# MiraPurkrabek/ProbPose_code

Measured on AMD Instinct MI355X. Metric: person-crops/sec @ 256x192 bs64, higher is better.
Workload: dtype f16x3

## Files before the change

include/probpose_mi355x.h:

```cpp
#ifndef PROBPOSE_MI355X_H_
#define PROBPOSE_MI355X_H_

#include <stddef.h>
#include <stdint.h>

#ifdef __cplusplus
extern "C" {
#endif

#define PP_ABI_VERSION 4


enum {
    PP_OK = 0,
    PP_ERR_INVALID_ARG = -1,
    PP_ERR_UNSUPPORTED = -2,
    PP_ERR_HIP = -3,
    PP_ERR_WORKSPACE = -4
};

#define PP_MAX_RADIUS 9
#define PP_MAX_TAPS (2 * PP_MAX_RADIUS + 1)

int pp_abi_version(void);
// ... 141 lines not shown

int pp_qkv_attention_split_folded(const void* x_centered, const void* wqkv_folded, const float* bqkv_folded, const float* ln_stats, void* out,
                                  int n_seq, int seq_len, int heads, int head_dim, float scale, float w_inv_scale, void* stream);

long long pp_proj_split_packed_bytes(int E);
int pp_proj_split_pack_weights(const void* wp_split, void* packed, int E, void* stream);
int pp_proj_ffn_split_residual_layernorm(const void* att, const void* wproj_packed, const float* bproj,
                                         const float* gamma2, const float* beta2, void* h_scratch, const void* w_packed,
                                         const float* b1, const float* b2, const float* residual, float* x_out,
                                         const float* gamma, const float* beta, float eps, void* h_out, int M, int E,
                                         int F, void* stream);
int pp_proj_ffn_split_residual_layernorm_ws(const void* att, const void* wproj_packed, const float* bproj,
                                            const float* gamma2, const float* beta2, void* h_scratch, const void* w_packed,
                                            const float* b1, const float* b2, const float* residual, float* x_out,
                                            const float* gamma, const float* beta, float eps, void* h_out, int M, int E,
                                            int F, float wp_inv_scale, float w1_inv_scale, float w2_inv_scale, void* stream);

int pp_proj_ffn_split_folded(const void* att, const void* wproj_packed, const float* bproj, const float* gamma2, const float* beta2,
                             void* h_scratch, const void* w_packed, const float* b1, const float* b2, const void* residual,
                             int residual_format, const float* residual_stats, int fold_out, float* x_out, const float* gamma,
                             const float* beta, float eps, void* h_out, float* stats_out, int M, int E, int F, float wp_inv_scale,
                             float w1_inv_scale, float w2_inv_scale, void* stream);

int pp_deconv_head(const void* act_nhwc, const void* weight, const float* bias, const void* head_w, const float* head_b,
                   float* logits_phased, int B, int H, int W, int Cin, int Cout, int K, void* stream);

int pp_deconv_head_split(const void* act_nhwc, const void* weight, const float* bias, const void* head_w_packed,
                         const float* head_b, float* logits_phased, int B, int H, int W, int Cin, int Cout, int K, void* stream);

int pp_probmap_head_decode_phased(const float* logits, const float* logits_flip, const int32_t* flip_indices,
                                  const double* taps, const int32_t* radius, int B, int K, int H, int W, double in_w,
                                  double in_h, float temperature, float normalize, float* avg_out, float* conv_out,
                                  float* locs, double* keypoints, float* scores, void* stream);

#define PP_DECODE_LOGITS 1
#define PP_DECODE_PHASED 2
#define PP_DECODE_SHIFT_HEATMAP 4
int pp_probmap_decode_flags(const float* maps, const float* maps_flip, const int32_t* flip_indices, const double* taps,
                            const int32_t* radius, int B, int K, int H, int W, double in_w, double in_h, float temperature,
                            float normalize, float* avg_out, float* conv_out, float* locs, double* keypoints, float* scores,
                            int flags, void* stream);

int pp_conv3x3_splitk(int prec, const void* act_nhwc, const void* weight, float* partials, int B, int H, int W, int Cin,
                      int Cout, int groups, long long stride_act_g, long long stride_w_g, int ksplit, void* stream);
int pp_sum_maxpool_relu_nhwc(const float* partials, int nsplit, long long split_stride, const float* bias,
                             int images_per_group, void* out, int out_bf16, int N, int H, int W, int C, int ph, int pw,
                             void* stream);

long long pp_winograd_scratch_bytes(int B, int H, int W, int Cin);
int pp_conv3x3_winograd_maxpool_relu(const void* act_nhwc, const void* u_packed, const float* bias, void* v_scratch,
                                     void* out_pooled, int B, int H, int W, int Cin, int Cout, int pool_h, int pool_w, int groups,
                                     void* stream);

int pp_tower_final(const void* feat, int feat_bf16, const float* w, const float* bias,
                   const int32_t* flip_indices, float* out, int B, int passes, int C, int K, float err_div,
                   void* stream);

int pp_extended_oks(const double* gt_kpts, const double* gt_bbox, const double* gt_area, const double* dt_kpts,
                    const double* sigmas, const int* gt_visibilities, int G, int D, int K, int n_vis,
                    double confidence_thr, double padding, int use_area, int original, double* out, void* stream);

int pp_pack_records(const double* keypoints, const float* scores, const float* scalars, double* records, int n, void* stream);

int pp_revert_heatmaps_max(const float* heatmaps, const double* inverse_maps, float* out, int n, int K, int hm_h, int hm_w,
                           int img_h, int img_w, void* stream);

int pp_heatmap_posterior(float* heatmaps, const float* presence, double* scratch, int K, int H, int W, void* stream);

int pp_exoks_cells(const double* gt_kpts, const double* gt_bbox, const double* gt_area, const double* dt_kpts,
                   const double* sigmas, const int* gt_visibilities, const int* cell_gt_off, const int* cell_dt_off,
                   const long long* cell_out_off, int n_cells, int K, int n_vis, double confidence_thr, double padding,
                   int use_area, int original, double* out, void* stream);

int pp_exoks_match(const double* ious, const int* cell_gt_off, const int* cell_dt_off, const long long* cell_iou_off,
                   const unsigned char* gt_ignore, const unsigned char* gt_iscrowd, const double* gt_area,
                   const double* gt_bbox, const double* dt_area, const double* dt_bbox, const double* area_rng,
                   const double* iou_thrs, int n_cells, int max_gt_per_cell, int N_gt, int N_dt, int L, int A, int T,
                   int match_by_bbox, int* dt_match, unsigned char* dt_ignore, int* gt_match,
                   unsigned char* gt_ignore_out, double* sim_sum, int* sim_cnt, void* stream);

int pp_exmap_accumulate(const int* dt_match, const unsigned char* dt_ignore, const unsigned char* gt_ignore,
                        const int* order, const double* dt_score, const double* rec_thrs, int n_cells, int N_gt, int N_dt,
                        int L, int A, int T, int R, int* chunk_scratch, double* precision, double* recall, double* scores,
                        void* stream);

int pp_warp_affine_u8(const void* img_hwc, int img_h, int img_w, int channels, const double* inverse_maps, void* crops_chw,
                      int n, int out_h, int out_w, void* stream);

long long pp_parea_scratch_bytes(int K, int H, int W);
int pp_parea_thresholds(const float* maps, int K, int H, int W, void* scratch, float* thr, int* draw, void* stream);
int pp_parea_compose(const void* image_rgb, int img_h, int img_w, int pad_left, int pad_top, const float* maps, int K,
                     const float* thr, const int* draw, const int* boxes, int n_boxes, void* canvas_rgb, int canvas_h,
                     int canvas_w, void* stream);
int pp_draw_poses(const void* image_rgb, int img_h, int img_w, const float* keypoints, const float* visible, const int* boxes,
                  int n, int K, const int* skeleton, const void* link_rgb, const void* kpt_rgb, int n_links, double kpt_thr,
                  float radius, float thickness, float alpha, void* out_rgb, void* stream);
int pp_resize_bilinear_u8(const void* src_rgb, int src_h, int src_w, void* dst_rgb, int dst_h, int dst_w, void* stream);

#ifdef __cplusplus
}
#endif
#endif
```

probpose_code_amd/_lib.py:

```python
import ctypes
import os
from ctypes import c_char_p, c_double, c_float, c_int, c_longlong, c_void_p

import torch

_HERE = os.path.dirname(os.path.abspath(__file__))
LIB_NAME = "libprobpose_mi355x.so"
LIB_PATH = os.path.join(_HERE, LIB_NAME)

PP_OK = 0
PP_ERR_INVALID_ARG = -1
PP_ERR_UNSUPPORTED = -2
PP_ERR_HIP = -3
PP_ERR_WORKSPACE = -4
PP_MAX_RADIUS = 9
PP_MAX_TAPS = 2 * PP_MAX_RADIUS + 1


class ProbPoseLibraryError(RuntimeError):

    def __init__(self, fn, status, message):
        super().__init__(f"{fn} failed with {status}: {message}")
        self.status = status

# ... 62 lines not shown
        [c_int, _P, _P, _P, _P, c_int, _P, _P, _P, c_float, _P, c_int, c_int, c_int, c_int, c_int, c_int, _P],
    ),
    "pp_gemm_residual_layernorm_ws": (
        c_int,
        [c_int, _P, _P, _P, _P, c_int, _P, _P, _P, c_float, _P, c_int, c_int, c_int, c_int, c_int, c_int, c_float, _P],
    ),
    "pp_mlp_residual_layernorm": (c_int, [_P, _P, _P, _P, _P, _P, _P, _P, _P, c_float, _P, c_int, c_int, c_int, _P]),
    "pp_proj_mlp_residual_layernorm": (
        c_int, [_P, _P, _P, _P, _P, _P, _P, _P, _P, _P, _P, _P, _P, c_float, _P, _P, _P, _P, c_int, c_int, c_int, _P]),
    "pp_vit_layer": (
        c_int, [_P, c_int, c_int, c_float, _P, _P, _P, _P, _P, _P, _P, _P, _P, _P, _P, _P, c_float, _P, _P, _P, _P, c_int, c_int,
                c_int, _P]),
    "pp_ffn_split_packed_bytes": (c_longlong, [c_int, c_int]),
    "pp_ffn_split_pack_weights": (c_int, [_P, _P, _P, c_int, c_int, _P]),
    "pp_ffn_split_residual_layernorm": (c_int, [_P, _P, _P, _P, _P, _P, _P, _P, c_float, _P, c_int, c_int, c_int, _P]),
    "pp_ffn_split_residual_layernorm_ws": (c_int, [_P, _P, _P, _P, _P, _P, _P, _P, c_float, _P, c_int, c_int, c_int, c_float, c_float, _P]),
    "pp_qkv_attention_split": (c_int, [_P, _P, _P, _P, c_int, c_int, c_int, c_int, c_float, _P]),
    "pp_qkv_attention_split_ws": (c_int, [_P, _P, _P, _P, c_int, c_int, c_int, c_int, c_float, c_float, _P]),
    "pp_qkv_attention_split_folded": (c_int, [_P] * 5 + [c_int] * 4 + [c_float, c_float, _P]),
    "pp_proj_split_packed_bytes": (c_longlong, [c_int]),
    "pp_proj_split_pack_weights": (c_int, [_P, _P, c_int, _P]),
    "pp_proj_ffn_split_residual_layernorm": (
        c_int, [_P, _P, _P, _P, _P, _P, _P, _P, _P, _P, _P, _P, _P, c_float, _P, c_int, c_int, c_int, _P]),
    "pp_proj_ffn_split_residual_layernorm_ws": (
        c_int, [_P, _P, _P, _P, _P, _P, _P, _P, _P, _P, _P, _P, _P, c_float, _P, c_int, c_int, c_int, c_float, c_float, c_float, _P]),
    "pp_proj_ffn_split_folded": (
        c_int, [_P] * 10 + [c_int, _P, c_int, _P, _P, _P, c_float, _P, _P, c_int, c_int, c_int, c_float, c_float, c_float, _P]),
    "pp_conv3x3_splitk": (c_int, [c_int, _P, _P, _P, c_int, c_int, c_int, c_int, c_int, c_int, c_longlong, c_longlong, c_int, _P]),
    "pp_sum_maxpool_relu_nhwc": (c_int, [_P, c_int, c_longlong, _P, c_int, _P, c_int, c_int, c_int, c_int, c_int, c_int, c_int, _P]),
    "pp_warp_affine_u8": (c_int, [_P, c_int, c_int, c_int, _P, _P, c_int, c_int, c_int, _P]),
    "pp_extended_oks": (
        c_int, [_P, _P, _P, _P, _P, _P, c_int, c_int, c_int, c_int, c_double, c_double, c_int, c_int, _P, _P]),
    "pp_pack_records": (c_int, [_P, _P, _P, _P, c_int, _P]),
    "pp_revert_heatmaps_max": (c_int, [_P, _P, _P] + [c_int] * 6 + [_P]),
    "pp_heatmap_posterior": (c_int, [_P, _P, _P, c_int, c_int, c_int, _P]),
    "pp_exoks_cells": (
        c_int, [_P] * 9 + [c_int, c_int, c_int, c_double, c_double, c_int, c_int, _P, _P]),
    "pp_exoks_match": (
        c_int, [_P] * 12 + [c_int] * 8 + [_P] * 7),
    "pp_exmap_accumulate": (
        c_int, [_P] * 6 + [c_int] * 7 + [_P] * 5),
    "pp_conv_gemm": (
        c_int,
        [c_int, c_int, _P, _P, _P, _P, c_int, c_int, c_int, c_int, c_int, c_int, c_int, c_int,
         c_longlong, c_longlong, c_longlong, c_longlong, c_int, c_int, c_int, _P],
    ),
    "pp_attention": (c_int, [c_int, _P, _P, c_int, c_int, c_int, c_int, c_float, _P]),
    "pp_preproc_im2col": (c_int, [c_int, _P, c_int, _P, c_int, c_int, c_int, c_int, c_int, c_int, _P, _P, c_int, _P]),
    "pp_layernorm": (c_int, [_P, _P, _P, _P, c_int, c_int, c_float, c_int, _P]),
    "pp_maxpool_relu_nhwc": (c_int, [_P, c_int, _P, c_int, c_int, c_int, c_int, c_int, c_int, c_int, _P]),
    "pp_conv3x3_maxpool_relu": (c_int, [c_int, _P, _P, _P, _P, _P] + [c_int] * 8 + [c_longlong] * 3 + [c_int, _P]),
    "pp_winograd_scratch_bytes": (c_longlong, [c_int] * 4),
    "pp_conv3x3_winograd_maxpool_relu": (c_int, [_P] * 5 + [c_int] * 8 + [_P]),
    "pp_tower_final": (c_int, [_P, c_int, _P, _P, _P, _P, c_int, c_int, c_int, c_int, c_float, _P]),
    "pp_parea_scratch_bytes": (c_longlong, [c_int, c_int, c_int]),
    "pp_parea_thresholds": (c_int, [_P, c_int, c_int, c_int, _P, _P, _P, _P]),
    "pp_parea_compose": (c_int, [_P, c_int, c_int, c_int, c_int, _P, c_int, _P, _P, _P, c_int, _P, c_int, c_int, _P]),
    "pp_draw_poses": (
        c_int, [_P, c_int, c_int, _P, _P, _P, c_int, c_int, _P, _P, _P, c_int, c_double, c_float, c_float, c_float, _P, _P]),
    "pp_resize_bilinear_u8": (c_int, [_P, c_int, c_int, _P, c_int, c_int, _P]),
}

for _name, (_res, _args) in SIGNATURES.items():
    _fn = getattr(lib, _name)
    _fn.restype = _res
    _fn.argtypes = _args


class PlanShape(ctypes.Structure):
    _fields_ = [(n, c_int) for n in ("prec", "n_img", "n_tokens", "embed", "ffn", "patch_k", "n_keypoints", "feat_h", "feat_w",
                                     "heat_h", "heat_w", "deconv_channels")]


WS = dict(patches=0, x=1, h=2, qkv=3, att=4, ln2=5, ffn=6, feat=7, logits=8, deconv=9, tower=10, tower_partial=11, tower_pooled=12, winograd=13, ln_stats=14)


def workspace_bytes(buffer: str, shape: "PlanShape", index: int = 0) -> int:
    n = lib.pp_workspace_bytes(WS[buffer], index, ctypes.byref(shape))
    if n < 0:
        raise ProbPoseLibraryError("pp_workspace_bytes", lib.pp_status_string(int(n)).decode(), last_error())
    return int(n)


_option_epoch = 0


_option_first_values = {}


def set_option(name: str, value: int) -> None:
    global _option_epoch
    if name not in _option_first_values:
        v = ctypes.c_int(0)
        if lib.pp_get_option(name.encode(), ctypes.byref(v)) == PP_OK:
            _option_first_values[name] = int(v.value)
    check("pp_set_option", lib.pp_set_option(name.encode(), int(value)))
    _option_epoch += 1


def restore_options() -> None:
    for name, v in list(_option_first_values.items()):
        if get_option(name) != v:
            set_option(name, v)


def option_epoch() -> int:
# ... 58 lines not shown
```

probpose_code_amd/engine.py:

```python
import math
import os
import warnings
from typing import Dict, Optional, Sequence

import numpy as np
import ctypes

import torch

from . import _lib
from .codecs import oks_kernel_taps
from .weights import PackedWeights, from_split, pack, to_split

PREC = {"bf16": 0, "f32": 1, "f16x3": 2}
_DTYPE = {"bf16": torch.bfloat16, "f32": torch.float32, "f16x3": torch.float32}
_FMT = {"bf16": 1, "f32": 0, "f16x3": 2}
ACT_NONE, ACT_GELU, ACT_RELU = 0, 1, 2
CONV3X3, DECONV = 1, 2


PLAN_DEFAULTS = dict(fuse_mlp=True, fuse_proj=True, fuse_qkv=True, split_k=True, fuse_attn=True, fuse_head=True, fuse_resln=None,
                     fuse_pool=True, fuse_qkv_attn=True, winograd=True, ln_fold=True, small_plan=True, head_two_streams=True)
SMALL_PLAN_ROWS_BELOW = 6912

# ... 99 lines not shown
            bp = torch.zeros(rows, dtype=torch.float32, device=fb.device)
            bp[: fb.shape[0]] = fb
            self._final_padded = (wp, bp)
        self.small_rows_below = SMALL_PLAN_ROWS_BELOW
        self.fuse_attn, self.fuse_head, self.fuse_pool = pl["fuse_attn"], pl["fuse_head"], pl["fuse_pool"]
        self.fuse_resln = pl["fuse_resln"] is not False
        self._resln_768 = pl["fuse_resln"] is True
        self._ffn_packed: Dict[int, torch.Tensor] = {}
        self._proj_packed: Dict[int, torch.Tensor] = {}
        if precision == "f16x3" and self.fuse_mlp and _lib.lib.pp_ffn_split_packed_bytes(self.E, self.w.ffn_dims) > 0:
            nbytes = _lib.lib.pp_ffn_split_packed_bytes(self.E, self.w.ffn_dims)
            pbytes = _lib.lib.pp_proj_split_packed_bytes(self.E) if self.fuse_proj else -1
            with torch.cuda.device(self.device):
                for i in range(self.w.num_layers):
                    buf = torch.empty(nbytes // 4, dtype=torch.float32, device=self.device)
                    _lib.call("pp_ffn_split_pack_weights", self.w[f"l{i}.fc1.w"].data_ptr(), self.w[f"l{i}.fc2.w"].data_ptr(),
                              buf.data_ptr(), self.E, self.w.ffn_dims, _lib.stream_ptr(self.device))
                    self._ffn_packed[i] = buf
                    if pbytes > 0:
                        pbuf = torch.empty(pbytes // 4, dtype=torch.float32, device=self.device)
                        _lib.call("pp_proj_split_pack_weights", self.w[f"l{i}.proj.w"].data_ptr(), pbuf.data_ptr(), self.E,
                                  _lib.stream_ptr(self.device))
                        self._proj_packed[i] = pbuf
                torch.cuda.synchronize(self.device)
            if not (pl["small_plan"]):
                for i in range(self.w.num_layers):
                    for name in (f"l{i}.fc1.w", f"l{i}.fc2.w") + ((f"l{i}.proj.w",) if i in self._proj_packed else ()):
                        self.w.t.pop(name, None)
        self.fuse_qkv_attn = precision == "f16x3" and pl["fuse_qkv_attn"] and self.Np == 192 and self.hd == 32 and self.E == 384
        self.ln_fold = bool(precision == "f16x3" and pl["ln_fold"] and not self._proj_packed and not self._ffn_packed
                            and self.w.has("l0.fc1.wf") and self.E % 192 == 0 and self.w.ffn_dims % 192 == 0)
        self.ln_fold_fused = bool(precision == "f16x3" and pl["ln_fold"] and self.fuse_qkv_attn and self._proj_packed and self.w.has("l1.qkv.wf")
                                  and (self.w.ffn_dims // 128) % 2 == 0 and self.w.num_layers >= 2)
        if precision == "f16x3":
            if self.fuse_qkv_attn and self._proj_packed:
                self.layer_plan = "two launches per layer (pp_qkv_attention_split + pp_proj_ffn_split_residual_layernorm)"
                if self.ln_fold_fused:
                    self.layer_plan += "; ln1 of layers 1 .. L - 1 folded into the qkv projection (pp_proj_ffn_split_folded -> pp_qkv_attention_split_folded)"
            elif self._proj_packed:
                self.layer_plan = "three launches per layer (pp_gemm qkv + pp_attention + pp_proj_ffn_split_residual_layernorm)"
            else:
                self.layer_plan = "generic (pp_gemm / pp_attention / pp_layernorm per layer)"
                if self.ln_fold:
                    self.layer_plan += ("; from the row count at which the twelve-wave Linear kernel engages: LayerNorm folded into the Linear "
                                        "layers (pp_linear_ln_folded x4 + pp_attention per layer, residual stream in the operand format)")
            if pl["fuse_qkv_attn"] and not self.fuse_qkv_attn and self.E == 384 and self.hd == 32:
                warnings.warn(
                    f"ProbPoseEngine: {self.Np}-token sequences ({img_size[0]}x{img_size[1]} input) miss the fused qkv + attention kernel, "
                    f"which is built for 192 tokens (256x192); this model runs {self.layer_plan}", RuntimeWarning, stacklevel=2)
        else:
            self.layer_plan = "bf16 / f32 plan"
        self.winograd = (precision == "f16x3" and pl["winograd"] and self.w.has("tower0.wino")
                         and _lib.lib.pp_winograd_scratch_bytes(1, self.Hp, self.Wp, self.E) > 0)
        if self.w.has("tower0.wino") and not self.winograd:
            self.w.t.pop("tower0.wino")
        self._logits_phased = False
        self._head_stream: Optional[torch.cuda.Stream] = None
        self._capture_events: list = []
        self._eager_events: dict = {}
        self.profile: Optional[Dict[str, list]] = None
        self.stage_hook = None
        self.pools = ((4, 3), (2, 2), (2, 2))
        hs, ws_ = self.Hp, self.Wp
        self.tower_hw = []
        for ph, pw_ in self.pools:
            self.tower_hw.append((hs, ws_))
            hs, ws_ = hs // ph, ws_ // pw_
        if (hs, ws_) != (1, 1):
            raise ValueError(
                f"scalar towers reduce the {self.Hp}x{self.Wp} feature map to {hs}x{ws_}; the reference "
                "reshapes them to (B, 1, K) (probmap_head.py:780-783), which needs 1x1"
            )

    def ksplit(self, nb: int, th: int, tw: int) -> int:
        return int(_lib.lib.pp_conv3x3_splitk_slices(self.prec, int(nb), int(th), int(tw), self.E, self.E, 4))

    def _workspace(self, B: int, passes: int, slot: int = 0) -> Dict[str, torch.Tensor]:
        self._check_options()
        key = (B, passes, slot)
        if key in self._ws:
            return self._ws[key]
        dev, T, f32 = self.device, self.dtype, torch.float32
        nb = B * passes
        M = nb * self.Np
        E, Fd = self.E, self.w.ffn_dims
        dc = self.w.deconv_channels
        shape = _lib.PlanShape(prec=self.prec, n_img=nb, n_tokens=self.Np, embed=E, ffn=Fd, patch_k=3 * self.P * self.P, n_keypoints=self.K,
                               feat_h=self.Hp, feat_w=self.Wp, heat_h=self.Hh, heat_w=self.Wh, deconv_channels=dc[0] if dc else 0)

        def buf(which, dims, dt=T, index=0):
            nbytes = _lib.workspace_bytes(which, shape, index)
            t = torch.empty(nbytes, dtype=torch.uint8, device=dev).view(dt)
            assert t.numel() == math.prod(dims), (which, index, nbytes, dims)
            return t.view(*dims)

        e = lambda *s, dt=T: torch.empty(s, dtype=dt, device=dev)
        small = self._small_at(M)
        fused_layer = self.precision == "f16x3" and self.fuse_qkv_attn and bool(self._proj_packed) and not small
        ws = dict(
            patches=buf("patches", (M, 3 * self.P * self.P)), x=buf("x", (M, E), f32), h=buf("h", (M, E)),
            feat=buf("feat", (M, E)), logits=buf("logits", (nb, self.K, self.Hh * self.Wh), f32),
            qkv=None if (fused_layer or (small and self.fuse_qkv_attn)) else buf("qkv", (M, 3 * E)),
            qkv2=None if (fused_layer or small) else buf("qkv", (M, 3 * E)),
            f=None if ((fused_layer or self._ffn_packed) and not small) else buf("ffn", (M, Fd)),
            att=buf("att", (M, E)) if (self.fuse_qkv_attn or small) else None,
            hs=buf("ln2", (M, E)) if (self._proj_packed or small) else None,
            ln_count=torch.zeros((M + 31) // 32, dtype=torch.int32, device=dev) if small else None,
            xs=buf("h", (M, E)) if self._ln_fold_at(M) else None,
# ... 243 lines not shown
            wj = w[f"deconv{j}.w"]
            if (j == nd - 1 and self.fuse_head and ob == 1 and cout == 256 and w.has("final.w_pad") and cin % 32 == 0
                    and ww % 4 == 0 and self.K <= 28):
                self._call("deconv_head", "pp_deconv_head", src.data_ptr(), wj.data_ptr(), w[f"deconv{j}.b"].data_ptr(),
                           w["final.w_pad"].data_ptr(), w["final.b"].data_ptr(), ws["logits"].data_ptr(), nb, hh, ww, cin, cout,
                           self.K, st)
                self._logits_phased = True
                return ws["logits"]
            if (j == nd - 1 and self.fuse_head and ob == 2 and cout == 256 and w.has("final.w_head") and cin % 32 == 0
                    and ww % 4 == 0 and self.K <= 28 and nb * hh * ww * 4 >= 192 * 192):
                self._call("deconv_head", "pp_deconv_head_split", src.data_ptr(), wj.data_ptr(), w[f"deconv{j}.b"].data_ptr(),
                           w["final.w_head"].data_ptr(), w["final.b"].data_ptr(), ws["logits"].data_ptr(), nb, hh, ww, cin, cout,
                           self.K, st)
                self._logits_phased = True
                return ws["logits"]
            if ob == 2 and self._small_at(nb * self.Np) and nb * hh * ww <= 1536 and cin % 32 == 0 and cout % 32 == 0:
                self._call("deconv", "pp_skinny_deconv", src.data_ptr(), wj.data_ptr(), w[f"deconv{j}.b"].data_ptr(), dst.data_ptr(), nb, hh, ww, cin,
                           cout, st)
                src, cin, hh, ww = dst, cout, hh * 2, ww * 2
                continue
            self._call("deconv", "pp_conv_gemm", self.prec, DECONV, src.data_ptr(), wj.data_ptr(),
                       w[f"deconv{j}.b"].data_ptr(), dst.data_ptr(), nb, hh, ww, cin, cout, -1, -1, 1, 0, 0, 0, 0, cout,
                       ACT_RELU, ob, st)
            src, cin, hh, ww = dst, cout, hh * 2, ww * 2
        P = hh * ww
        if ob == 2 and self._small_at(nb * self.Np) and cin % 64 == 0 and self._final_padded is not None:
            wp, bp = self._final_padded
            self._call("final_conv", "pp_skinny_conv1x1_planar", src.data_ptr(), wp.data_ptr(), bp.data_ptr(), ws["logits"].data_ptr(), nb, P, cin, self.K,
                       w.inv("final.w"), st)
            return ws["logits"]
        self._gemm(st, src, w["final.w"], w["final.b"], ws["logits"], nb * P, self.K, cin, planar=P, out_bf16=0)
        return ws["logits"]

    def towers(self, feat: torch.Tensor, B: int, passes: int, flip_indices, ws, st) -> torch.Tensor:
        w, E = self.w, self.E
        nb = B * passes
        ob = self.fmt
        src, stride_src = feat, 0
        for j, (th, tw) in enumerate(self.tower_hw):
            ph, pw_ = self.pools[j]
            out = ws[f"t{j}"]
            rows = nb * th * tw
            if self.split_k and f"tp{j}" in ws:
                part = ws[f"tp{j}"]
                ks = part.shape[0]
                self._call("conv3x3_splitk", "pp_conv3x3_splitk", self.prec, src.data_ptr(), w[f"tower{j}.w"].data_ptr(),
                           part.data_ptr(), nb, th, tw, E, E, 4, stride_src, E * 9 * E, ks, st)
                self._call("maxpool", "pp_sum_maxpool_relu_nhwc", part.data_ptr(), ks, 4 * rows * E, w[f"tower{j}.b"].data_ptr(),
                           nb, ws[f"p{j}"].data_ptr(), ob, 4 * nb, th, tw, E, ph, pw_, st)
                src = ws[f"p{j}"]
                stride_src = nb * (th // ph) * (tw // pw_) * E
                continue
            if j == 0 and self.winograd and ws.get("wino") is not None and stride_src == 0 and (ph, pw_) == (4, 3):
                self._call("conv3x3", "pp_conv3x3_winograd_maxpool_relu", src.data_ptr(), w["tower0.wino"].data_ptr(), w["tower0.b"].data_ptr(),
                           ws["wino"].data_ptr(), ws["p0"].data_ptr(), nb, th, tw, E, E, ph, pw_, 4, st)
            elif self.fuse_pool:
                self._call("conv3x3", "pp_conv3x3_maxpool_relu", self.prec, src.data_ptr(), w[f"tower{j}.w"].data_ptr(),
                           w[f"tower{j}.b"].data_ptr(), ws[f"p{j}"].data_ptr(), out.data_ptr(), nb, th, tw, E, E, ph, pw_, 4,
                           stride_src, E * 9 * E, E, ob, st)
            else:
                self._call("conv3x3", "pp_conv_gemm", self.prec, CONV3X3, src.data_ptr(), w[f"tower{j}.w"].data_ptr(),
                           w[f"tower{j}.b"].data_ptr(), out.data_ptr(), nb, th, tw, E, E, 0, 0, 4, stride_src,
                           E * 9 * E, nb * th * tw * E, E, E, ACT_NONE, ob, st)
                self._call("maxpool", "pp_maxpool_relu_nhwc", out.data_ptr(), ob, ws[f"p{j}"].data_ptr(), ob, 4 * nb, th, tw, E, ph,
                           pw_, st)
            src = ws[f"p{j}"]
            stride_src = nb * (th // ph) * (tw // pw_) * E
        fi = self._flip_indices(flip_indices) if passes == 2 else None
        self._call("tower_final", "pp_tower_final", src.data_ptr(), ob, w["tower_out.w"].data_ptr(), w["tower_out.b"].data_ptr(),
                  _lib.ptr(fi), ws["scalars"].data_ptr(), B, passes, E, self.K, 1.0, st)
        return ws["scalars"]

    def _check_imgs(self, imgs: torch.Tensor):
        assert imgs.dim() == 4 and imgs.is_cuda, "expects a (B,3,H,W) tensor on the GPU"
        assert imgs.dtype in (torch.uint8, torch.float32), "crops are uint8 (raw) or float32 (already preprocessed)"
        assert tuple(imgs.shape[1:]) == (3, self.H, self.W), f"crop shape {tuple(imgs.shape)} != (B,3,{self.H},{self.W})"

    @torch.no_grad()
    def run_backbone(self, imgs: torch.Tensor, flip_test: bool, slot: int = 0) -> torch.Tensor:
        self._check_imgs(imgs)
        imgs = imgs.contiguous()
        B, passes = imgs.shape[0], 2 if flip_test else 1
        ws = self._workspace(B, passes, slot)
        with torch.cuda.device(self.device):
            feat = self.backbone(imgs, passes, ws, _lib.stream_ptr(self.device))
        return feat.view(B * passes, self.Hp, self.Wp, self.E)

    def export_features(self, feat: torch.Tensor) -> torch.Tensor:
        return from_split(feat) if self.precision == "f16x3" else feat.clone()

    def import_features(self, x_nhwc: torch.Tensor) -> torch.Tensor:
        if self.precision == "f16x3":
            return to_split(x_nhwc.float().contiguous())
        if x_nhwc.dtype != self.dtype or not x_nhwc.is_contiguous():
            x_nhwc = x_nhwc.to(self.dtype).contiguous()
        return x_nhwc

    @torch.no_grad()
    def run_head(self, feat_nhwc: torch.Tensor, flip_test: bool, flip_indices=None,
                 return_heatmaps: bool = False, slot: int = 0, shift_heatmap: bool = False) -> Dict[str, torch.Tensor]:
        passes = 2 if flip_test else 1
        nb = feat_nhwc.shape[0]
        assert nb % passes == 0 and tuple(feat_nhwc.shape[1:]) == (self.Hp, self.Wp, self.E)
        assert feat_nhwc.dtype == self.dtype and feat_nhwc.is_contiguous() and feat_nhwc.is_cuda
        if flip_test and flip_indices is None:
            raise ValueError("flip_test needs flip_indices (dataset meta)")
        B = nb // passes
        ws = self._workspace(B, passes, slot)
# ... 171 lines not shown
```

probpose_code_amd/weights.py:

```python
import math
from dataclasses import dataclass, field
from typing import Dict, List

import torch

TOWERS = ("probability", "visibility", "oks", "error")
BN_EPS = 1e-5


def to_split(x: torch.Tensor) -> torch.Tensor:
    K = x.shape[-1]
    assert K % 32 == 0, f"split-fp16 tensors need a last dimension that is a multiple of 32, got {K}"
    x = x.float()
    hi = x.half()
    lo = (x - hi.float()).half()
    lead = x.shape[:-1]
    blocks = torch.stack([hi.reshape(*lead, K // 32, 32), lo.reshape(*lead, K // 32, 32)], dim=-2)
    return blocks.reshape(*lead, 2 * K).contiguous().view(torch.float32)


def from_split(c: torch.Tensor) -> torch.Tensor:
    K = c.shape[-1]
    v = c.contiguous().view(torch.float16).reshape(*c.shape[:-1], K // 32, 2, 32).float()
    return (v[..., 0, :] + v[..., 1, :]).reshape(c.shape)
# ... 72 lines not shown


@dataclass
class PackedWeights:
    dtype: torch.dtype
    embed_dims: int
    num_layers: int
    ffn_dims: int
    num_keypoints: int
    deconv_channels: List[int]
    t: Dict[str, torch.Tensor] = field(default_factory=dict)
    inv_scale: Dict[str, float] = field(default_factory=dict)

    def __getitem__(self, k):
        return self.t[k]

    def inv(self, k) -> float:
        return float(self.inv_scale.get(k, 1.0))

    def has(self, k) -> bool:
        return k in self.t


def _bn_fold(sd, name):
    scale = sd[name + ".weight"].float() / torch.sqrt(sd[name + ".running_var"].float() + BN_EPS)
    shift = sd[name + ".bias"].float() - sd[name + ".running_mean"].float() * scale
    return scale, shift


def pack_head_split(w32: torch.Tensor) -> torch.Tensor:
    assert tuple(w32.shape) == (32, 256)
    w32 = w32.float()
    hi = w32.half()
    lo = (w32 - hi.float()).half()
    lane = torch.arange(64)
    fr, fg = lane % 16, lane // 16
    j = torch.arange(8)
    ch_in_blk = torch.where(j < 4, 4 * fg[:, None] + j[None, :], 16 + 4 * fg[:, None] + (j[None, :] - 4))
    out = torch.empty((4, 2, 2, 2, 64, 8), dtype=torch.float16)
    for cg in range(4):
        for kb in range(2):
            ch = 64 * cg + 32 * kb + ch_in_blk
            for nf in range(2):
                rows = (16 * nf + fr)[:, None].expand(64, 8)
                out[cg, kb, nf, 0] = hi[rows, ch]
                out[cg, kb, nf, 1] = lo[rows, ch]
    return out.reshape(-1).view(torch.float32).contiguous()


def winograd_weights(w: torch.Tensor) -> torch.Tensor:
    G = torch.tensor([[1.0, 0.0, 0.0], [0.5, 0.5, 0.5], [0.5, -0.5, 0.5], [0.0, 0.0, 1.0]], dtype=torch.float64)
    u = torch.einsum("ai,ocij,bj->aboc", G, w.double(), G)
    return u.reshape(16, w.shape[0], w.shape[1]).float()


def pack(sd: Dict[str, torch.Tensor], dtype: torch.dtype, device, split: bool = False, scale_linear: bool = True,
         num_heads: int = 0, fold_ln: bool = True) -> PackedWeights:
    sd = {k: v.detach().cpu() for k, v in normalize_state_dict(sd).items()}
    if split and scale_linear and num_heads > 0:
        n_layers = 1 + max(int(k.split(".")[2]) for k in sd if k.startswith("backbone.layers."))
        for i in range(n_layers):
            if sd[f"backbone.layers.{i}.attn.qkv.weight"].shape[1] % num_heads == 0:
                balance_attention_dims(sd, f"backbone.layers.{i}.", num_heads)
    f32 = lambda x: x.float().contiguous().to(device)
    inv_scale: Dict[str, float] = {}
    if split:
        def op(x, name="weights", scaled=False):
            check_split_range(name, x)
            x = x.float()
            if scaled and scale_linear:
                e = weight_scale_exponent(x)
                x = x * 2.0 ** e
                inv_scale[name] = 2.0 ** -e
            return to_split(x.contiguous()).to(device)
    else:
        op = lambda x, name=None, scaled=False: x.float().contiguous().to(dtype).to(device)
    pw = sd["backbone.patch_embed.projection.weight"]
    E = pw.shape[0]
    L = 1 + max(int(k.split(".")[2]) for k in sd if k.startswith("backbone.layers."))
    Fd = sd["backbone.layers.0.ffn.layers.0.0.weight"].shape[0]
    K = sd["head.final_layer.weight"].shape[0]
    t: Dict[str, torch.Tensor] = {}
    t["patch_w"] = op(pw.reshape(E, -1), "patch_w")
    t["patch_b"] = f32(sd["backbone.patch_embed.projection.bias"])
    t["pos_embed"] = f32(sd["backbone.pos_embed"].reshape(-1, E))
    for i in range(L):
        p = f"backbone.layers.{i}."
        for ln in ("ln1", "ln2"):
            t[f"l{i}.{ln}.w"] = f32(sd[p + ln + ".weight"])
            t[f"l{i}.{ln}.b"] = f32(sd[p + ln + ".bias"])
        t[f"l{i}.qkv.w"] = op(sd[p + "attn.qkv.weight"], f"l{i}.qkv.w", scaled=True)
        qb = sd.get(p + "attn.qkv.bias")
        t[f"l{i}.qkv.b"] = f32(qb if qb is not None else torch.zeros(3 * E))
        t[f"l{i}.proj.w"] = op(sd[p + "attn.proj.weight"], f"l{i}.proj.w", scaled=True)
        t[f"l{i}.proj.b"] = f32(sd[p + "attn.proj.bias"])
        t[f"l{i}.fc1.w"] = op(sd[p + "ffn.layers.0.0.weight"], f"l{i}.fc1.w", scaled=True)
        t[f"l{i}.fc1.b"] = f32(sd[p + "ffn.layers.0.0.bias"])
        t[f"l{i}.fc2.w"] = op(sd[p + "ffn.layers.1.weight"], f"l{i}.fc2.w", scaled=True)
        t[f"l{i}.fc2.b"] = f32(sd[p + "ffn.layers.1.bias"])
        if split and fold_ln and E == 384 and i >= 1:
            bb = sd.get(p + "attn.qkv.bias")
            e = weight_scale_exponent(sd[p + "attn.qkv.weight"].double() * sd[p + "ln1.weight"].double()[None, :]) if scale_linear else 0
            wf, _, bf = fold_layernorm(sd[p + "attn.qkv.weight"].float(), bb.float() if bb is not None else torch.zeros(3 * E),
                                       sd[p + "ln1.weight"].float(), sd[p + "ln1.bias"].float(), name=f"l{i}.qkv.wf", scale_exp=e)
            t[f"l{i}.qkv.wf"], t[f"l{i}.qkv.bf"] = wf.to(device), bf.to(device)
            inv_scale[f"l{i}.qkv.wf"] = 2.0 ** -e
        if split and fold_ln and E % 192 == 0 and E != 384:
            for name, wk, bk, ln in (("qkv", "attn.qkv.weight", "attn.qkv.bias", "ln1"), ("fc1", "ffn.layers.0.0.weight", "ffn.layers.0.0.bias", "ln2")):
                bb = sd.get(p + bk)
                e = weight_scale_exponent(sd[p + wk].double() * sd[p + ln + ".weight"].double()[None, :]) if scale_linear else 0
                wf, cs, bf = fold_layernorm(sd[p + wk].float(), bb.float() if bb is not None else torch.zeros(sd[p + wk].shape[0]),
                                            sd[p + ln + ".weight"].float(), sd[p + ln + ".bias"].float(), name=f"l{i}.{name}.wf", scale_exp=e)
                t[f"l{i}.{name}.wf"], t[f"l{i}.{name}.cf"], t[f"l{i}.{name}.bf"] = wf.to(device), cs.to(device), bf.to(device)
                inv_scale[f"l{i}.{name}.wf"] = 2.0 ** -e
    t["ln_f.w"] = f32(sd["backbone.ln1.weight"])
    t["ln_f.b"] = f32(sd["backbone.ln1.bias"])

    deconv_channels = []
    j = 0
    while f"head.deconv_layers.{3 * j}.weight" in sd:
        w = sd[f"head.deconv_layers.{3 * j}.weight"].float()
        assert w.shape[2:] == (4, 4), "only deconv kernel 4 / stride 2 / pad 1 (the ProbPose config) is packed"
        scale, shift = _bn_fold(sd, f"head.deconv_layers.{3 * j + 1}")
        w = w * scale.view(1, -1, 1, 1)
        cin, cout = w.shape[:2]
        ph = torch.empty((2, 2, cout, 4 * cin))
        for py in range(2):
            for px in range(2):
                for ty in range(2):
                    for tx in range(2):
                        tap = ty * 2 + tx
                        ph[py, px, :, tap * cin : (tap + 1) * cin] = w[:, :, 3 - 2 * ty - py, 3 - 2 * tx - px].t()
        t[f"deconv{j}.w"] = op(ph, f"deconv{j}.w")
        t[f"deconv{j}.b"] = f32(shift)
        deconv_channels.append(cout)
        j += 1
    t["final.w"] = op(sd["head.final_layer.weight"].reshape(K, -1), "final.w")
    t["final.b"] = f32(sd["head.final_layer.bias"])
    if K <= 32:
        wpad = torch.zeros((32, t["final.w"].shape[1]), dtype=torch.float32)
        wpad[:K] = sd["head.final_layer.weight"].reshape(K, -1).float()
        t["final.w_pad"] = op(wpad, "final.w_pad")
        if split and wpad.shape[1] == 256:
            t["final.w_head"] = pack_head_split(wpad).to(device)

    for c in range(3):
        ws, bs, wino = [], [], []
        for tw in TOWERS:
            base = f"head.{tw}_layers."
            w = sd[base + f"{4 * c}.weight"].float()
            b = sd[base + f"{4 * c}.bias"].float()
            scale, shift = _bn_fold(sd, base + f"{4 * c + 1}")
            w = w * scale.view(-1, 1, 1, 1)
            ws.append(w.permute(0, 2, 3, 1).reshape(w.shape[0], -1))
            bs.append(b * scale + shift)
            if c == 0 and split:
                wino.append(winograd_weights(w))
        if c == 0 and split and w.shape[1] % 128 == 0 and w.shape[0] % 96 == 0:
            t["tower0.wino"] = op(torch.stack(wino), "tower0.wino")
        t[f"tower{c}.w"] = op(torch.stack(ws), f"tower{c}.w")
        t[f"tower{c}.b"] = f32(torch.stack(bs))
    t["tower_out.w"] = f32(torch.stack([sd[f"head.{tw}_layers.12.weight"].float().reshape(K, -1) for tw in TOWERS]))
    t["tower_out.b"] = f32(torch.stack([sd[f"head.{tw}_layers.12.bias"].float() for tw in TOWERS]))
    return PackedWeights(dtype=dtype, embed_dims=E, num_layers=L, ffn_dims=Fd, num_keypoints=K,
                         deconv_channels=deconv_channels, t=t, inv_scale=inv_scale)
```

Before: 14700.

## Add Winograd F(4x3,3x3) conv with fused maxpool for first tower layer

Adds a new Winograd variant whose output tile matches the (4,3) maxpool window, using 30 transform points instead of 16 per 2x2 tile. The output transform is folded into the GEMM epilogue so each pooled output is produced directly. The intent is fewer multiplies per output pixel and less scratch traffic for the first tower conv than the existing F(2x2) path. The trade-offs are larger transform coefficients with a numerical accuracy risk in split-f16 precision, and more accumulator registers.

```diff
diff --git a/include/probpose_mi355x.h b/include/probpose_mi355x.h
--- a/include/probpose_mi355x.h
+++ b/include/probpose_mi355x.h
@@ -217,6 +217,11 @@
                                      void* out_pooled, int B, int H, int W, int Cin, int Cout, int pool_h, int pool_w, int groups,
                                      void* stream);
 
+long long pp_winograd43_scratch_bytes(int B, int H, int W, int Cin);
+int pp_conv3x3_winograd43_maxpool_relu(const void* act_nhwc, const void* u_packed, const float* bias, void* v_scratch,
+                                       void* out_pooled, int B, int H, int W, int Cin, int Cout, int pool_h, int pool_w, int groups,
+                                       void* stream);
+
 int pp_tower_final(const void* feat, int feat_bf16, const float* w, const float* bias,
                    const int32_t* flip_indices, float* out, int B, int passes, int C, int K, float err_div,
                    void* stream);
diff --git a/probpose_code_amd/_lib.py b/probpose_code_amd/_lib.py
--- a/probpose_code_amd/_lib.py
+++ b/probpose_code_amd/_lib.py
@@ -138,6 +138,8 @@
     "pp_conv3x3_maxpool_relu": (c_int, [c_int, _P, _P, _P, _P, _P] + [c_int] * 8 + [c_longlong] * 3 + [c_int, _P]),
     "pp_winograd_scratch_bytes": (c_longlong, [c_int] * 4),
     "pp_conv3x3_winograd_maxpool_relu": (c_int, [_P] * 5 + [c_int] * 8 + [_P]),
+    "pp_winograd43_scratch_bytes": (c_longlong, [c_int] * 4),
+    "pp_conv3x3_winograd43_maxpool_relu": (c_int, [_P] * 5 + [c_int] * 8 + [_P]),
     "pp_tower_final": (c_int, [_P, c_int, _P, _P, _P, _P, c_int, c_int, c_int, c_int, c_float, _P]),
     "pp_parea_scratch_bytes": (c_longlong, [c_int, c_int, c_int]),
     "pp_parea_thresholds": (c_int, [_P, c_int, c_int, c_int, _P, _P, _P, _P]),
diff --git a/probpose_code_amd/csrc/pp_winograd43.hip b/probpose_code_amd/csrc/pp_winograd43.hip
--- /dev/null
+++ b/probpose_code_amd/csrc/pp_winograd43.hip
@@ -0,0 +1,341 @@
+#include "pp_common.h"
+#include "pp_split.h"
+
+namespace pp {
+namespace wino43 {
+
+typedef float f32x4 __attribute__((ext_vector_type(4)));
+typedef unsigned int u32x4 __attribute__((ext_vector_type(4)));
+typedef __attribute__((address_space(3))) void* lds_ptr_t;
+
+constexpr int PH = 4, PW = 3;
+constexpr int NP = 30;
+constexpr int RF = 2, CF = 3;
+constexpr int BT = 32 * RF, BN = 32 * CF, THREADS = 256;
+constexpr int NST = 4;
+constexpr unsigned OOB = 0x7ffffff0u;
+
+struct Params {
+    const void* V;
+    const void* U;
+    const float* bias;
+    void* out;
+    int T, Cin, Cout, groups;
+    int order;
+    unsigned v_bytes, u_bytes;
+};
+
+__device__ __forceinline__ f32x4 mma(const u32x4& a, const u32x4& b, f32x4 c) {
+    return __builtin_amdgcn_mfma_f32_16x16x32_f16(__builtin_bit_cast(f16x8, a), __builtin_bit_cast(f16x8, b), c, 0, 0, 0);
+}
+
+template <int N>
+__device__ __forceinline__ void wait_vm_lgkm() {
+    __builtin_amdgcn_s_waitcnt((N & 15) | (7 << 4) | (0 << 8) | ((N >> 4) << 14));
+}
+
+__device__ __forceinline__ float atr(int i, int a) {
+    if (a == 0) return i == 0 ? 1.f : 0.f;
+    if (a == 5) return i == 3 ? 1.f : 0.f;
+    const float x = a == 1 ? 1.f : (a == 2 ? -1.f : (a == 3 ? 0.5f : -0.5f));
+    return i == 0 ? 1.f : (i == 1 ? x : (i == 2 ? x * x : x * x * x));
+}
+__device__ __forceinline__ float atc(int j, int b) {
+    if (b == 0) return j == 0 ? 1.f : 0.f;
+    if (b == 4) return j == 2 ? 1.f : 0.f;
+    const float x = b == 1 ? 1.f : (b == 2 ? -1.f : 0.5f);
+    return j == 0 ? 1.f : (j == 1 ? x : x * x);
+}
+
+__global__ __launch_bounds__(256) void input_transform_kernel(const char* __restrict__ feat, char* __restrict__ V, int nb, int C, int H, int W) {
+    const int G4 = C >> 2;
+    const long long idx = (long long)blockIdx.x * blockDim.x + threadIdx.x;
+    const int TX = W / 3, TY = H / 4;
+    const long long T = (long long)nb * TY * TX;
+    if (idx >= T * G4) return;
+    const int g4 = (int)(idx % G4);
+    const long long tile = idx / G4;
+    const int tx = (int)(tile % TX), ty = (int)((tile / TX) % TY), img = (int)(tile / ((long long)TX * TY));
+    const int boff = (g4 >> 3) * 128 + (g4 & 7) * 8;
+    f32x4 e[6][5];
+#pragma unroll
+    for (int r = 0; r < 6; ++r) {
+        f32x4 d[5];
+#pragma unroll
+        for (int c = 0; c < 5; ++c) {
+            const int y = 4 * ty - 1 + r, x = 3 * tx - 1 + c;
+            f32x4 v = {0.f, 0.f, 0.f, 0.f};
+            if (y >= 0 && y < H && x >= 0 && x < W) {
+                const char* src = feat + ((size_t)(img * H + y) * W + x) * (size_t)(C * 4) + boff;
+                const f16x4 h = *reinterpret_cast<const f16x4*>(src), l = *reinterpret_cast<const f16x4*>(src + 64);
+#pragma unroll
+                for (int j = 0; j < 4; ++j) v[j] = (float)h[j] + (float)l[j];
+            }
+            d[c] = v;
+        }
+        e[r][0] = 0.5f * d[0] - d[1] - 0.5f * d[2] + d[3];
+        e[r][1] = -0.5f * d[1] + 0.5f * d[2] + d[3];
+        e[r][2] = 0.5f * d[1] - 1.5f * d[2] + d[3];
+        e[r][3] = d[3] - d[1];
+        e[r][4] = 0.5f * d[1] - d[2] - 0.5f * d[3] + d[4];
+    }
+#pragma unroll
+    for (int b = 0; b < 5; ++b) {
+        f32x4 o[6];
+        o[0] = 0.25f * e[0][b] - 1.25f * e[2][b] + e[4][b];
+        o[1] = -0.25f * e[1][b] - 0.25f * e[2][b] + e[3][b] + e[4][b];
+        o[2] = 0.25f * e[1][b] - 0.25f * e[2][b] - e[3][b] + e[4][b];
+        o[3] = -0.5f * e[1][b] - e[2][b] + 0.5f * e[3][b] + e[4][b];
+        o[4] = 0.5f * e[1][b] - e[2][b] - 0.5f * e[3][b] + e[4][b];
+        o[5] = 0.25f * e[1][b] - 1.25f * e[3][b] + e[5][b];
+#pragma unroll
+        for (int a = 0; a < 6; ++a) {
+            f16x4 h, l;
+#pragma unroll
+            for (int j = 0; j < 4; ++j) {
+                h[j] = split_hi(o[a][j]);
+                l[j] = split_lo(o[a][j], h[j]);
+            }
+            char* dst = V + ((size_t)(5 * a + b) * (size_t)T + (size_t)tile) * (size_t)(C * 4) + boff;
+            *reinterpret_cast<f16x4*>(dst) = h;
+            *reinterpret_cast<f16x4*>(dst + 64) = l;
+        }
+    }
+}
+
+__global__ __launch_bounds__(THREADS, 1) void gemm_pool_kernel(const Params p) {
+    constexpr int STAGE = (BT + BN) * 128;
+    constexpr int NPW = (BT + BN) / 32;
+    extern __shared__ __attribute__((aligned(16))) char smem[];
+    const int tid = threadIdx.x, lane = tid & 63;
+    const int wv = __builtin_amdgcn_readfirstlane(tid >> 6);
+    const int cg = wv >> 1, rg = wv & 1;
+    const int fr = lane & 15, fg = lane >> 4;
+    const int sw = fr & 7;
+
+    const int CT = p.groups * (p.Cout / BN);
+    const int RB = (p.T + BT - 1) / BT;
+    int id = blockIdx.x;
+    const int nblk = gridDim.x;
+    if ((nblk & 7) == 0) id = (id & 7) * (nblk >> 3) + (id >> 3);
+    int ct, rb;
+    const int sc = p.order;
+    if (sc > 0) {
+        const int sr = 32 / sc, st = id >> 5, w = id & 31, sct = st % (CT / sc), srb = st / (CT / sc);
+        rb = sr * srb + w / sc;
+        ct = sc * sct + w % sc;
+    } else {
+        ct = id % CT;
+        rb = id / CT;
+    }
+    if (rb >= RB) return;
+    const int g = (ct * BN) / p.Cout, n0 = ct * BN - g * p.Cout;
+    const int KB = p.Cin >> 5;
+    const int nstages = NP * KB;
+
+    const int d_l = lane >> 3;
+    const unsigned d_sw = (unsigned)(((lane & 7) ^ d_l) << 4);
+    const __amdgpu_buffer_rsrc_t v_rsrc = __builtin_amdgcn_make_buffer_rsrc(const_cast<void*>(p.V), 0, p.v_bytes, 0x00020000);
+    const __amdgpu_buffer_rsrc_t u_rsrc = __builtin_amdgcn_make_buffer_rsrc(const_cast<void*>(p.U), 0, p.u_bytes, 0x00020000);
+    const unsigned rowb = (unsigned)(p.Cin * 4);
+    const unsigned v_v = (unsigned)(rb * BT + 8 * wv + d_l) * rowb + d_sw;
+    const unsigned v_u = (unsigned)((g * NP) * p.Cout + n0 + 8 * wv + d_l) * rowb + d_sw;
+    const unsigned v_pstride = (unsigned)p.T * rowb, u_pstride = (unsigned)p.Cout * rowb;
+    int i_s = 0, i_p = 0, i_kb = 0;
+    auto issue_stage = [&]() {
+        char* dst = smem + (i_s & (NST - 1)) * STAGE + wv * 1024;
+        const bool live = i_s < nstages;
+        const unsigned so_v = __builtin_amdgcn_readfirstlane(live ? (unsigned)i_p * v_pstride + (unsigned)(i_kb * 128) : OOB);
+        const unsigned so_u = __builtin_amdgcn_readfirstlane(live ? (unsigned)i_p * u_pstride + (unsigned)(i_kb * 128) : OOB);
+#pragma unroll
+        for (int j = 0; j < RF; ++j)
+            __builtin_amdgcn_raw_ptr_buffer_load_lds(v_rsrc, (lds_ptr_t)(dst + j * 4096), 16, live ? v_v + (unsigned)(j * 32) * rowb : OOB, live ? so_v : 0, 0, 0);
+#pragma unroll
+        for (int j = 0; j < CF; ++j)
+            __builtin_amdgcn_raw_ptr_buffer_load_lds(u_rsrc, (lds_ptr_t)(dst + BT * 128 + j * 4096), 16, live ? v_u + (unsigned)(j * 32) * rowb : OOB, live ? so_u : 0, 0, 0);
+        ++i_s;
+        if (++i_kb == KB) {
+            i_kb = 0;
+            ++i_p;
+        }
+    };
+
+    const int a_off = (32 * rg + fr) * 128, w_off = BT * 128 + (16 * CF * cg + fr) * 128;
+    const int ch_hi = (fg ^ sw) << 4, ch_lo = ((4 + fg) ^ sw) << 4;
+    auto frag_a = [&](int buf, int lo, int rf) -> u32x4 {
+        return *reinterpret_cast<const u32x4*>(smem + buf * STAGE + a_off + rf * 2048 + (lo ? ch_lo : ch_hi));
+    };
+    auto frag_w = [&](int buf, int lo, int cf) -> u32x4 {
+        return *reinterpret_cast<const u32x4*>(smem + buf * STAGE + w_off + cf * 2048 + (lo ? ch_lo : ch_hi));
+    };
+
+    f32x4 tmp[CF][RF], P[3][CF][RF], Y[12][CF][RF];
+#pragma unroll
+    for (int cf = 0; cf < CF; ++cf)
+#pragma unroll
+        for (int rf = 0; rf < RF; ++rf) {
+            tmp[cf][rf] = f32x4{0.f, 0.f, 0.f, 0.f};
+#pragma unroll
+            for (int j = 0; j < 3; ++j) P[j][cf][rf] = f32x4{0.f, 0.f, 0.f, 0.f};
+#pragma unroll
+            for (int o = 0; o < 12; ++o) Y[o][cf][rf] = f32x4{0.f, 0.f, 0.f, 0.f};
+        }
+#pragma unroll
+    for (int s = 0; s < NST; ++s) issue_stage();
+    wait_vm_lgkm<3 * NPW>();
+    __builtin_amdgcn_s_barrier();
+    u32x4 ah[RF], wh[CF], al[RF], wl[CF];
+#pragma unroll
+    for (int cf = 0; cf < CF; ++cf) wh[cf] = frag_w(0, 0, cf);
+#pragma unroll
+    for (int rf = 0; rf < RF; ++rf) ah[rf] = frag_a(0, 0, rf);
+
+#pragma unroll 1
+    for (int pos = 0; pos < NP; ++pos) {
+#pragma unroll 1
+        for (int kq = 0; kq < KB; kq += NST) {
+#pragma unroll
+            for (int u = 0; u < NST; ++u) {
+                const int cb = u, nb = (u + 1) & (NST - 1);
+                __builtin_amdgcn_sched_barrier(0);
+#pragma unroll
+                for (int cf = 0; cf < CF; ++cf) wl[cf] = frag_w(cb, 1, cf);
+#pragma unroll
+                for (int rf = 0; rf < RF; ++rf) al[rf] = frag_a(cb, 1, rf);
+#pragma unroll
+                for (int rf = 0; rf < RF; ++rf)
+#pragma unroll
+                    for (int cf = 0; cf < CF; ++cf) tmp[cf][rf] = mma(wh[cf], ah[rf], tmp[cf][rf]);
+                __builtin_amdgcn_sched_barrier(0);
+                wait_vm_lgkm<2 * NPW>();
+                __builtin_amdgcn_s_barrier();
+                __builtin_amdgcn_sched_barrier(0);
+                issue_stage();
+#pragma unroll
+                for (int rf = 0; rf < RF; ++rf) {
+#pragma unroll
+                    for (int cf = 0; cf < CF; ++cf) tmp[cf][rf] = mma(wl[cf], ah[rf], tmp[cf][rf]);
+                    ah[rf] = frag_a(nb, 0, rf);
+                }
+#pragma unroll
+                for (int cf = 0; cf < CF; ++cf) {
+#pragma unroll
+                    for (int rf = 0; rf < RF; ++rf) tmp[cf][rf] = mma(wh[cf], al[rf], tmp[cf][rf]);
+                    wh[cf] = frag_w(nb, 0, cf);
+                }
+            }
+        }
+        const int a = pos / 5, b = pos - 5 * (pos / 5);
+#pragma unroll
+        for (int j = 0; j < 3; ++j) {
+            const float c = atc(j, b);
+            if (c != 0.f) {
+#pragma unroll
+                for (int cf = 0; cf < CF; ++cf)
+#pragma unroll
+                    for (int rf = 0; rf < RF; ++rf)
+#pragma unroll
+                        for (int q = 0; q < 4; ++q) P[j][cf][rf][q] = __builtin_fmaf(tmp[cf][rf][q], c, P[j][cf][rf][q]);
+            }
+        }
+#pragma unroll
+        for (int cf = 0; cf < CF; ++cf)
+#pragma unroll
+            for (int rf = 0; rf < RF; ++rf) tmp[cf][rf] = f32x4{0.f, 0.f, 0.f, 0.f};
+        if (b == 4) {
+#pragma unroll
+            for (int i = 0; i < 4; ++i) {
+                const float c = atr(i, a);
+                if (c != 0.f) {
+#pragma unroll
+                    for (int j = 0; j < 3; ++j)
+#pragma unroll
+                        for (int cf = 0; cf < CF; ++cf)
+#pragma unroll
+                            for (int rf = 0; rf < RF; ++rf)
+#pragma unroll
+                                for (int q = 0; q < 4; ++q) Y[3 * i + j][cf][rf][q] = __builtin_fmaf(P[j][cf][rf][q], c, Y[3 * i + j][cf][rf][q]);
+                }
+            }
+#pragma unroll
+            for (int j = 0; j < 3; ++j)
+#pragma unroll
+                for (int cf = 0; cf < CF; ++cf)
+#pragma unroll
+                    for (int rf = 0; rf < RF; ++rf) P[j][cf][rf] = f32x4{0.f, 0.f, 0.f, 0.f};
+        }
+    }
+    wait_vm_lgkm<0>();
+#pragma unroll
+    for (int cf = 0; cf < CF; ++cf) {
+        const int ch = n0 + 16 * CF * cg + 16 * cf + 4 * fg;
+        f32x4 bv = {0.f, 0.f, 0.f, 0.f};
+        if (p.bias) bv = *reinterpret_cast<const f32x4*>(p.bias + (size_t)g * p.Cout + ch);
+#pragma unroll
+        for (int rf = 0; rf < RF; ++rf) {
+            const int t = rb * BT + 32 * rg + 16 * rf + fr;
+            f32x4 m = Y[0][cf][rf];
+#pragma unroll
+            for (int o = 1; o < 12; ++o)
+#pragma unroll
+                for (int q = 0; q < 4; ++q) m[q] = fmaxf(m[q], Y[o][cf][rf][q]);
+            f32x4 r;
+#pragma unroll
+            for (int q = 0; q < 4; ++q) r[q] = fmaxf(m[q] + bv[q], 0.f);
+            if (t < p.T) split_store4(p.out, ((size_t)g * p.T + t) * (size_t)p.Cout + ch, r);
+        }
+    }
+}
+
+}
+}
+
+extern "C" long long pp_winograd43_scratch_bytes(int B, int H, int W, int Cin) {
+    using namespace pp;
+    if (B <= 0 || H <= 0 || W <= 0 || H % 4 != 0 || W % 3 != 0 || Cin <= 0 || Cin % 128 != 0) return PP_ERR_UNSUPPORTED;
+    return 30ll * B * (H / 4) * (W / 3) * Cin * 4;
+}
+
+extern "C" int pp_conv3x3_winograd43_maxpool_relu(const void* act_nhwc, const void* u_packed, const float* bias, void* v_scratch,
+                                                  void* out_pooled, int B, int H, int W, int Cin, int Cout, int pool_h, int pool_w,
+                                                  int groups, void* stream) {
+    using namespace pp;
+    PP_REQUIRE(act_nhwc && u_packed && v_scratch && out_pooled, PP_ERR_INVALID_ARG, "pp_conv3x3_winograd43_maxpool_relu: NULL argument");
+    PP_REQUIRE(B > 0 && groups >= 1, PP_ERR_INVALID_ARG, "pp_conv3x3_winograd43_maxpool_relu: bad B / groups");
+    PP_REQUIRE(H > 0 && W > 0 && H % 4 == 0 && W % 3 == 0 && pool_h == wino43::PH && pool_w == wino43::PW, PP_ERR_UNSUPPORTED,
+               "pp_conv3x3_winograd43_maxpool_relu: built for feature maps with H % 4 == 0, W % 3 == 0 pooled (4, 3)");
+    PP_REQUIRE(Cin % 128 == 0 && Cout % wino43::BN == 0, PP_ERR_UNSUPPORTED,
+               "pp_conv3x3_winograd43_maxpool_relu: Cin must be a multiple of 128, Cout of 96");
+    const long long T = (long long)B * (H / 4) * (W / 3);
+    const long long vb = 30ll * T * Cin * 4, ub = 30ll * groups * Cout * (long long)Cin * 4;
+    PP_REQUIRE(vb < wino43::OOB && ub < wino43::OOB && (long long)groups * T * Cout < (1ll << 40), PP_ERR_UNSUPPORTED,
+               "pp_conv3x3_winograd43_maxpool_relu: operands must be smaller than 2 GiB");
+    hipStream_t s = reinterpret_cast<hipStream_t>(stream);
+    const long long items = T * (Cin / 4);
+    hipLaunchKernelGGL(wino43::input_transform_kernel, dim3((unsigned)((items + 255) / 256)), dim3(256), 0, s,
+                       reinterpret_cast<const char*>(act_nhwc), reinterpret_cast<char*>(v_scratch), B, Cin, H, W);
+    PP_LAUNCH_CHECK_AS("winograd_input_transform");
+    wino43::Params p{};
+    p.V = v_scratch;
+    p.U = u_packed;
+    p.bias = bias;
+    p.out = out_pooled;
+    p.T = (int)T;
+    p.Cin = Cin;
+    p.Cout = Cout;
+    p.groups = groups;
+    p.v_bytes = (unsigned)vb;
+    p.u_bytes = (unsigned)ub;
+    const long long ct_ = (long long)groups * (Cout / wino43::BN), rb_ = (T + wino43::BT - 1) / wino43::BT;
+    int order = option("wino_order");
+    if (order < 0 || order > 32 || (order & (order - 1)) != 0 || (order > 0 && ct_ % order != 0)) order = 0;
+    p.order = order;
+    const long long sr_ = order > 0 ? 32 / order : 1;
+    const long long grid = ((rb_ + sr_ - 1) / sr_) * sr_ * ct_;
+    PP_REQUIRE(grid < (1ll << 30), PP_ERR_UNSUPPORTED, "pp_conv3x3_winograd43_maxpool_relu: too many tiles");
+    constexpr int lds = wino43::NST * (wino43::BT + wino43::BN) * 128;
+    PP_HIP_CHECK(hipFuncSetAttribute(reinterpret_cast<const void*>(wino43::gemm_pool_kernel), hipFuncAttributeMaxDynamicSharedMemorySize, lds));
+    hipLaunchKernelGGL(wino43::gemm_pool_kernel, dim3((unsigned)grid), dim3(wino43::THREADS), lds, s, p);
+    PP_LAUNCH_CHECK_AS("winograd_gemm_pool");
+    return PP_OK;
+}
diff --git a/probpose_code_amd/engine.py b/probpose_code_amd/engine.py
--- a/probpose_code_amd/engine.py
+++ b/probpose_code_amd/engine.py
@@ -175,8 +175,12 @@
             self.layer_plan = "bf16 / f32 plan"
         self.winograd = (precision == "f16x3" and pl["winograd"] and self.w.has("tower0.wino")
                          and _lib.lib.pp_winograd_scratch_bytes(1, self.Hp, self.Wp, self.E) > 0)
-        if self.w.has("tower0.wino") and not self.winograd:
-            self.w.t.pop("tower0.wino")
+        n43 = _lib.lib.pp_winograd43_scratch_bytes(1, self.Hp, self.Wp, self.E) if self.winograd else -1
+        self.winograd43 = (self.winograd and self.w.has("tower0.wino43") and 0 < n43 <= _lib.lib.pp_winograd_scratch_bytes(1, self.Hp, self.Wp, self.E)
+                           and self.E % 96 == 0)
+        for name, used in (("tower0.wino", self.winograd and not self.winograd43), ("tower0.wino43", self.winograd43)):
+            if self.w.has(name) and not used:
+                self.w.t.pop(name)
         self._logits_phased = False
         self._head_stream: Optional[torch.cuda.Stream] = None
         self._capture_events: list = []
@@ -526,8 +530,12 @@
                 stride_src = nb * (th // ph) * (tw // pw_) * E
                 continue
             if j == 0 and self.winograd and ws.get("wino") is not None and stride_src == 0 and (ph, pw_) == (4, 3):
-                self._call("conv3x3", "pp_conv3x3_winograd_maxpool_relu", src.data_ptr(), w["tower0.wino"].data_ptr(), w["tower0.b"].data_ptr(),
-                           ws["wino"].data_ptr(), ws["p0"].data_ptr(), nb, th, tw, E, E, ph, pw_, 4, st)
+                if self.winograd43:
+                    self._call("conv3x3", "pp_conv3x3_winograd43_maxpool_relu", src.data_ptr(), w["tower0.wino43"].data_ptr(),
+                               w["tower0.b"].data_ptr(), ws["wino"].data_ptr(), ws["p0"].data_ptr(), nb, th, tw, E, E, ph, pw_, 4, st)
+                else:
+                    self._call("conv3x3", "pp_conv3x3_winograd_maxpool_relu", src.data_ptr(), w["tower0.wino"].data_ptr(),
+                               w["tower0.b"].data_ptr(), ws["wino"].data_ptr(), ws["p0"].data_ptr(), nb, th, tw, E, E, ph, pw_, 4, st)
             elif self.fuse_pool:
                 self._call("conv3x3", "pp_conv3x3_maxpool_relu", self.prec, src.data_ptr(), w[f"tower{j}.w"].data_ptr(),
                            w[f"tower{j}.b"].data_ptr(), ws[f"p{j}"].data_ptr(), out.data_ptr(), nb, th, tw, E, E, ph, pw_, 4,
diff --git a/probpose_code_amd/weights.py b/probpose_code_amd/weights.py
--- a/probpose_code_amd/weights.py
+++ b/probpose_code_amd/weights.py
@@ -148,6 +148,24 @@
     G = torch.tensor([[1.0, 0.0, 0.0], [0.5, 0.5, 0.5], [0.5, -0.5, 0.5], [0.0, 0.0, 1.0]], dtype=torch.float64)
     u = torch.einsum("ai,ocij,bj->aboc", G, w.double(), G)
     return u.reshape(16, w.shape[0], w.shape[1]).float()
+
+
+WINO43_G_ROWS = ((4.0, 0.0, 0.0), (2 / 3, 2 / 3, 2 / 3), (2 / 3, -2 / 3, 2 / 3), (-8 / 3, -4 / 3, -2 / 3), (-8 / 3, 4 / 3, -2 / 3), (0.0, 0.0, 1.0))
+WINO43_G_COLS = ((2.0, 0.0, 0.0), (1.0, 1.0, 1.0), (-1 / 3, 1 / 3, -1 / 3), (-8 / 3, -4 / 3, -2 / 3), (0.0, 0.0, 1.0))
+WINO43_BT_ROWS = ((0.25, 0, -1.25, 0, 1, 0), (0, -0.25, -0.25, 1, 1, 0), (0, 0.25, -0.25, -1, 1, 0), (0, -0.5, -1, 0.5, 1, 0),
+                  (0, 0.5, -1, -0.5, 1, 0), (0, 0.25, 0, -1.25, 0, 1))
+WINO43_BT_COLS = ((0.5, -1, -0.5, 1, 0), (0, -0.5, 0.5, 1, 0), (0, 0.5, -1.5, 1, 0), (0, -1, 0, 1, 0), (0, 0.5, -1, -0.5, 1))
+WINO43_AT_ROWS = ((1, 1, 1, 1, 1, 0), (0, 1, -1, 0.5, -0.5, 0), (0, 1, 1, 0.25, 0.25, 0), (0, 1, -1, 0.125, -0.125, 1))
+WINO43_AT_COLS = ((1, 1, 1, 1, 0), (0, 1, -1, 0.5, 0), (0, 1, 1, 0.25, 1))
+WINO43_POINTS_ROWS = (0.0, 1.0, -1.0, 0.5, -0.5)
+WINO43_POINTS_COLS = (0.0, 1.0, -1.0, 0.5)
+
+
+def winograd43_weights(w: torch.Tensor) -> torch.Tensor:
+    Gr = torch.tensor(WINO43_G_ROWS, dtype=torch.float64)
+    Gc = torch.tensor(WINO43_G_COLS, dtype=torch.float64)
+    u = torch.einsum("ai,ocij,bj->aboc", Gr, w.double(), Gc)
+    return u.reshape(30, w.shape[0], w.shape[1]).float()
 
 
 def pack(sd: Dict[str, torch.Tensor], dtype: torch.dtype, device, split: bool = False, scale_linear: bool = True,
@@ -241,7 +259,7 @@
             t["final.w_head"] = pack_head_split(wpad).to(device)
 
     for c in range(3):
-        ws, bs, wino = [], [], []
+        ws, bs, wino, wino43 = [], [], [], []
         for tw in TOWERS:
             base = f"head.{tw}_layers."
             w = sd[base + f"{4 * c}.weight"].float()
@@ -252,8 +270,10 @@
             bs.append(b * scale + shift)
             if c == 0 and split:
                 wino.append(winograd_weights(w))
+                wino43.append(winograd43_weights(w))
         if c == 0 and split and w.shape[1] % 128 == 0 and w.shape[0] % 96 == 0:
             t["tower0.wino"] = op(torch.stack(wino), "tower0.wino")
+            t["tower0.wino43"] = op(torch.stack(wino43), "tower0.wino43")
         t[f"tower{c}.w"] = op(torch.stack(ws), f"tower{c}.w")
         t[f"tower{c}.b"] = f32(torch.stack(bs))
     t["tower_out.w"] = f32(torch.stack([sd[f"head.{tw}_layers.12.weight"].float().reshape(K, -1) for tw in TOWERS]))
```

Measured after the change: 14820 (median of 6 runs). Within noise of the previous version (+0.9%).
